# KogarashiNetwork/dusk-plonk

Measured on AMD Instinct MI355X. Metric: PLONK prover constraints/sec (BLS12-381) at n=2^16 and 2^20, 1/2/4/8 GPUs, higher is better.
Workload: dtype u32-limb Montgomery Fr/Fp (integer)

## Files before the change

### dusk-plonk_amd/csrc/debug.hip

```cpp
#include <hip/hip_runtime.h>

#include <algorithm>
#include <vector>

#include "g1r.hpp"
#include "internal.hpp"
#include "prover.hpp"

namespace plk {
namespace {

template <class C>
__global__ void k_field_op(int op, const Fe<C>* __restrict__ a, const Fe<C>* __restrict__ b,
                           Fe<C>* __restrict__ out, uint64_t n) {
  const uint64_t i = (uint64_t)blockIdx.x * blockDim.x + threadIdx.x;
  if (i >= n) return;
  const Fe<C> x = a[i], y = b[i];
  Fe<C> r;
  switch (op) {
    case 0: r = fe_mul(x, y); break;
    case 1: r = fe_add(x, y); break;
    case 2: r = fe_sub(x, y); break;
    case 3: r = fe_sqr(x); break;
    default: r = fe_inv(x); break;
// ... 91 lines not shown
  else if constexpr (OP == kOpSmall2) o0 = rx_small_mul_n<C, 2>(x0);
  else if constexpr (OP == kOpSmall3) o0 = rx_small_mul_n<C, 3>(x0);
  else if constexpr (OP == kOpCanon) o0 = rx_canon(x0);
  else if constexpr (OP == kOpIsZero) o0 = rx_flag<C>(rx_is_zero(x0));
  else if constexpr (OP == kOpIsZeroU) o0 = rx_flag<C>(rx_is_zero_u(x0));
  else if constexpr (OP == kOpUnpackPack) {
    Fe<C> w;
#pragma unroll
    for (int k = 0; k < C::N; ++k) w.v[k] = x0.v[k];
    o0 = rx_unpack(w);
    w = rx_pack(o0);
#pragma unroll
    for (int k = 0; k < C::N; ++k) o1.v[k] = w.v[k];
  } else if constexpr (OP >= kOpSubN) o0 = rx_sub_n<C, OP - kOpSubN>(x0, x1);
  else o0 = rx_sub_u<C, OP - kOpSubU>(x0, x1);
  st_row<C>(out, i * NOUT, o0);
  if constexpr (NOUT > 1) st_row<C>(out, i * NOUT + 1, o1);
  if constexpr (NOUT > 2) st_row<C>(out, i * NOUT + 2, o2);
}

using RxKernel = void (*)(const uint32_t*, const uint32_t*, const uint32_t*, const uint32_t*,
                          uint32_t*, uint64_t);
#define PLK_RX_CASE(C, OP) \
  case OP: return k_rx_op<C, OP>;
#define PLK_RX_COMMON(C)                                                                       \
  PLK_RX_CASE(C, kOpMul) PLK_RX_CASE(C, kOpSqr) PLK_RX_CASE(C, kOpMulAdd) PLK_RX_CASE(C, kOpMul2) \
  PLK_RX_CASE(C, kOpMul2Asm) PLK_RX_CASE(C, kOpSqr2) PLK_RX_CASE(C, kOpMulAddMul2)             \
  PLK_RX_CASE(C, kOpMul3) PLK_RX_CASE(C, kOpAdd) PLK_RX_CASE(C, kOpSub) PLK_RX_CASE(C, kOpSubLazy) \
  PLK_RX_CASE(C, kOpSub2N6) PLK_RX_CASE(C, kOpSmall2) PLK_RX_CASE(C, kOpSmall3)                \
  PLK_RX_CASE(C, kOpCanon) PLK_RX_CASE(C, kOpIsZero) PLK_RX_CASE(C, kOpIsZeroU)                \
  PLK_RX_CASE(C, kOpUnpackPack) PLK_RX_CASE(C, kOpSubU + 3) PLK_RX_CASE(C, kOpSubU + 5)        \
  PLK_RX_CASE(C, kOpSubU + 6) PLK_RX_CASE(C, kOpSubN + 3) PLK_RX_CASE(C, kOpSubN + 5)          \
  PLK_RX_CASE(C, kOpSubN + 6)
RxKernel rx_kernel(int field, int op) {
  if (field == 0) {
    switch (op) {
      PLK_RX_COMMON(FrCfg)
      default: return nullptr;
    }
  }
  switch (op) {
    PLK_RX_COMMON(FpCfg)
    PLK_RX_CASE(FpCfg, kOpSqr2Asm) PLK_RX_CASE(FpCfg, kOpMulAddMul2Asm)
    PLK_RX_CASE(FpCfg, kOpSubU + 4) PLK_RX_CASE(FpCfg, kOpSubU + 10)
    PLK_RX_CASE(FpCfg, kOpSubN + 4) PLK_RX_CASE(FpCfg, kOpSubN + 10)
    default: return nullptr;
  }
}
#undef PLK_RX_COMMON
#undef PLK_RX_CASE

enum : int {
  kG1Madd000 = 0, kG1Madd100, kG1Madd110, kG1Madd111, kG1MaddLazy, kG1AddLazy, kG1AddQuad,
  kG1DblLazy, kG1LazyFinish, kG1Add, kG1AddAffine, kG1Dbl, kG1DblAffine, kG1OpCount
};
constexpr int kG1Row = 4 * RxShape<FpCfg>::L;
constexpr bool g1_op_needs_q(int op) {
  return !(op == kG1DblLazy || op == kG1LazyFinish || op == kG1Dbl || op == kG1DblAffine);
}

__device__ __forceinline__ G1R ld_g1row(const uint32_t* __restrict__ p, uint64_t i) {
  G1R r;
  r.X = ld_row<FpCfg>(p, 4 * i);
  r.Y = ld_row<FpCfg>(p, 4 * i + 1);
  r.ZZ = ld_row<FpCfg>(p, 4 * i + 2);
  r.ZZZ = ld_row<FpCfg>(p, 4 * i + 3);
  return r;
}

template <bool GROUPED, bool ASM, bool PAIRS>
__device__ __forceinline__ G1R madd_as_accumulate(const G1R& acc, const G1R& q, bool neg) {
  RFp y = q.Y;
  if (neg) y = rx_neg_lazy(y);
  const bool was_inf = g1r_is_inf(acc);
  G1R r = g1r_madd_lazy_sl<GROUPED, ASM, PAIRS>(acc, q.X, y);
  if (rx_is_zero(r.ZZ)) {
    RFp yr = q.Y;
    if (neg) yr = rx_neg(yr);
    r = g1r_madd_lazy_fix(was_inf, r, q.X, yr);
  }
  return r;
}

template <int OP>
__global__ void __launch_bounds__(256)
    k_g1r_op(const uint32_t* __restrict__ p, const uint32_t* __restrict__ q,
             const uint32_t* __restrict__ flags, uint32_t* __restrict__ out, uint64_t n) {
  const uint64_t t = (uint64_t)blockIdx.x * blockDim.x + threadIdx.x;
  const uint64_t i = OP == kG1AddQuad ? t >> 2 : t;
  if (i >= n) return;
  const G1R a = ld_g1row(p, i);
  G1R b = g1_op_needs_q(OP) ? ld_g1row(q, i) : a;
  const bool neg = g1_op_needs_q(OP) && flags && (flags[i] & 1u);
  G1R r;
  if constexpr (OP == kG1Madd000) r = madd_as_accumulate<false, false, false>(a, b, neg);
  else if constexpr (OP == kG1Madd100) r = madd_as_accumulate<true, false, false>(a, b, neg);
  else if constexpr (OP == kG1Madd110) r = madd_as_accumulate<true, true, false>(a, b, neg);
  else if constexpr (OP == kG1Madd111) r = madd_as_accumulate<true, true, true>(a, b, neg);
  else if constexpr (OP == kG1MaddLazy) r = g1r_madd_lazy(a, b.X, neg ? rx_neg_lazy(b.Y) : b.Y);
  else if constexpr (OP == kG1AddLazy || OP == kG1AddQuad) {
    if (neg) b.Y = rx_neg_lazy(b.Y);
    if constexpr (OP == kG1AddLazy) r = g1r_add_lazy(a, b);
    else r = g1r_add_quad(a, b, threadIdx.x & 3u);
  } else if constexpr (OP == kG1DblLazy) r = g1r_dbl_lazy(a);
  else if constexpr (OP == kG1LazyFinish) r = g1r_lazy_finish(a);
  else if constexpr (OP == kG1Add) r = g1r_add(a, neg ? g1r_neg(b) : b);
  else if constexpr (OP == kG1AddAffine) r = g1r_add_affine(a, b.X, neg ? rx_neg(b.Y) : b.Y);
  else if constexpr (OP == kG1Dbl) r = g1r_dbl(a);
  else r = g1r_dbl_affine(a.X, a.Y);
  st_row<FpCfg>(out, 4 * t, r.X);
  st_row<FpCfg>(out, 4 * t + 1, r.Y);
  st_row<FpCfg>(out, 4 * t + 2, r.ZZ);
  st_row<FpCfg>(out, 4 * t + 3, r.ZZZ);
}

using G1Kernel = void (*)(const uint32_t*, const uint32_t*, const uint32_t*, uint32_t*, uint64_t);
G1Kernel g1r_kernel(int op) {
  switch (op) {
#define PLK_G1_CASE(OP) \
  case OP: return k_g1r_op<OP>;
    PLK_G1_CASE(kG1Madd000) PLK_G1_CASE(kG1Madd100) PLK_G1_CASE(kG1Madd110)
    PLK_G1_CASE(kG1Madd111) PLK_G1_CASE(kG1MaddLazy) PLK_G1_CASE(kG1AddLazy)
    PLK_G1_CASE(kG1AddQuad) PLK_G1_CASE(kG1DblLazy) PLK_G1_CASE(kG1LazyFinish)
    PLK_G1_CASE(kG1Add) PLK_G1_CASE(kG1AddAffine) PLK_G1_CASE(kG1Dbl) PLK_G1_CASE(kG1DblAffine)
#undef PLK_G1_CASE
    default: return nullptr;
  }
}

struct RowArg {
  const uint32_t* host;
  size_t bytes;
};
template <class K, size_t NA>
int run_rows(plk_ctx* ctx, K kern, const RowArg (&in)[NA], uint32_t* out, size_t out_bytes,
             uint64_t threads, uint64_t n) {
  DevBuf din[NA], dout;
  int st;
  hipStream_t s = ctx->stream;
  for (size_t k = 0; k < NA; ++k) {
    if (!in[k].host) continue;
    if ((st = din[k].alloc(in[k].bytes))) return st;
    PLK_HIP_TRY(hipMemcpyAsync(din[k].ptr, in[k].host, in[k].bytes, hipMemcpyHostToDevice, s));
  }
  if ((st = dout.alloc(out_bytes))) return st;
  const dim3 grid((unsigned)((threads + 255) / 256)), block(256);
  const uint32_t* dp[NA];
  for (size_t k = 0; k < NA; ++k) dp[k] = static_cast<const uint32_t*>(din[k].ptr);
  uint32_t* const dres = static_cast<uint32_t*>(dout.ptr);
  if constexpr (NA == 4)
    hipLaunchKernelGGL(kern, grid, block, 0, s, dp[0], dp[1], dp[2], dp[3], dres, n);
  else
    hipLaunchKernelGGL(kern, grid, block, 0, s, dp[0], dp[1], dp[2], dres, n);
  PLK_HIP_TRY(hipGetLastError());
  PLK_HIP_TRY(hipMemcpyAsync(out, dout.ptr, out_bytes, hipMemcpyDeviceToHost, s));
  PLK_HIP_TRY(stream_wait(s));
  return PLK_OK;
}


enum : int {
  kStPermNumDen = 0, kStScan, kStQuotient, kStPiSparse, kStPiCoef, kStCosetCombine, kStEval,
  kStLinComb, kStScalePowers, kStRuffini, kStCount
};

struct StageCall {
  int stage;
  const uint64_t* const* in;
  const size_t* len;
  size_t n_in;
  const plk_fr* sc;
  size_t n_sc;
  const uint64_t* par;
  size_t n_par;
  uint64_t* out;
  size_t out_cap;
};
// ... 296 lines not shown
```

### dusk-plonk_amd/csrc/ffr.hpp

```cpp
#pragma once
#include <type_traits>
#include <utility>

#include "ff.hpp"

namespace plk {

template <class C>
struct RxShape;
template <>
struct RxShape<FpCfg> {
  static constexpr int L = 13, B = 30;
  static constexpr uint32_t ONE[12] = {0x00d1ff2eu, 0x46760000u, 0x9b4800acu, 0x84b80337u,
                                       0xe882431cu, 0x0dd9a7e0u, 0xb683dcf8u, 0xc26c26d0u,
                                       0x63c4a5eeu, 0x29f14576u, 0x7f3e804bu, 0x015de996u};
};
template <>
struct RxShape<FrCfg> {
  static constexpr int L = 9, B = 29;
  static constexpr uint32_t ONE[8] = {0xffffffbau, 0x00000045u, 0x0072d846u, 0x1a25272eu,
                                      0x5dbeee8bu, 0xfe2eedcdu, 0x9eefbe41u, 0x4d043f42u};
};

template <class C>
// ... 55 lines not shown
  static constexpr int TOP_BITS = 26;
  bool split[2 * L - 1];
  constexpr RxPlan() : split{} {
    constexpr RxConst<C> K = RxK<C>::k;
    long double carry = 0;
    for (int k = 0; k < 2 * L - 1; ++k) {
      long double sum = carry;
      for (int i = 0; i < L; ++i) {
        const int j = k - i;
        if (j < 0 || j >= L) continue;
        const long double ai = (long double)(1ull << (i == L - 1 ? TOP_BITS : B));
        const long double bj = (long double)(1ull << (j == L - 1 ? TOP_BITS : B));
        sum += NPROD * ai * bj + (long double)(1ull << B) * (long double)(K.p[j] + 1);
      }
      split[k] = sum >= 18446744073709551616.0L;
      carry = sum / (long double)(1ull << B) + 4;
    }
  }
};
template <class C, int NPROD>
struct RxPlanK {
  static constexpr RxPlan<C, NPROD> k{};
};
template <class C>
struct RxMultiple {
  uint32_t v[RxShape<C>::L];
};

template <class C>
constexpr RxMultiple<C> rx_multiple(uint32_t c, bool borrow_free) {
  constexpr int L = RxShape<C>::L, B = RxShape<C>::B, N = C::N;
  uint32_t w[N + 1] = {};
  uint64_t carry = 0;
  for (int i = 0; i < N; ++i) {
    const uint64_t t = (uint64_t)C::P[i] * c + carry;
    w[i] = (uint32_t)t;
    carry = t >> 32;
  }
  w[N] = (uint32_t)carry;
  RxMultiple<C> m{};
  for (int i = 0; i < L; ++i) m.v[i] = rx_limb_of(w, N + 1, i, B, L);
  if (borrow_free) {
    m.v[0] += 1u << B;
    for (int i = 1; i < L - 1; ++i) m.v[i] += (1u << B) - 1;
    m.v[L - 1] -= 1;
  }
  return m;
}

template <class C, uint32_t CP, bool BF>
struct RxMultipleK {
  static constexpr RxMultiple<C> k = rx_multiple<C>(CP, BF);
};
static_assert(RxMultiple<FpCfg>{rx_multiple<FpCfg>(12, false)}.v[RxShape<FpCfg>::L - 1] <
                  (1u << RxPlan<FpCfg, 1>::TOP_BITS),
              "12p exceeds the split plan's operand bound");

#define PLK_RX __device__ __forceinline__

PLK_RX void rx_madd(uint64_t& acc, uint32_t x, uint32_t y) { acc += (uint64_t)x * y; }

template <class C>
PLK_RX void rx_column_close(bool split, int k, uint64_t& acc, uint64_t s2, uint64_t s3,
                            uint32_t* m, Rx<C>& r) {
  constexpr int L = RxShape<C>::L, B = RxShape<C>::B;
  constexpr uint32_t MASK = (1u << B) - 1;
  constexpr RxConst<C> K = RxK<C>::k;
  if (!split) {
    if (k < L) {
      m[k] = ((uint32_t)acc * K.inv) & MASK;
      rx_madd(acc, m[k], K.p[0]);
    } else {
      r.v[k - L] = (uint32_t)acc & MASK;
    }
    acc >>= B;
    return;
  }
  const uint32_t lo32 = ((uint32_t)acc & MASK) + ((uint32_t)s2 & MASK) + ((uint32_t)s3 & MASK);
  const uint64_t hi = (acc >> B) + (s2 >> B) + (s3 >> B);
  uint64_t lo = lo32;
  if (k < L) {
    m[k] = (lo32 * K.inv) & MASK;
    lo += (uint64_t)m[k] * K.p[0];
  } else {
    r.v[k - L] = lo32 & MASK;
  }
  acc = hi + (lo >> B);
}

template <class C>
PLK_RX Rx<C> rx_zero() {
  Rx<C> r;
#pragma unroll
  for (int i = 0; i < RxShape<C>::L; ++i) r.v[i] = 0;
  return r;
}

template <class C>
PLK_RX Rx<C> rx_one() {
  constexpr RxConst<C> K = RxK<C>::k;
  Rx<C> r;
#pragma unroll
  for (int i = 0; i < RxShape<C>::L; ++i) r.v[i] = K.one[i];
  return r;
}

template <class C>
// ... 737 lines not shown
```

### dusk-plonk_amd/csrc/g1r.hpp

```cpp
#pragma once
#include "ffr.hpp"
#include "g1.hpp"

namespace plk {

using RFp = Rx<FpCfg>;

struct G1R {
  RFp X, Y, ZZ, ZZZ;
};

__device__ __forceinline__ G1R g1r_infinity() {
  G1R r;
  r.X = rx_one<FpCfg>();
  r.Y = rx_one<FpCfg>();
  r.ZZ = rx_zero<FpCfg>();
  r.ZZZ = rx_zero<FpCfg>();
  return r;
}

__device__ __forceinline__ bool g1r_is_inf(const G1R& p) { return rx_is_zero(p.ZZ); }

__device__ __forceinline__ G1R g1r_neg(const G1R& p) {
  G1R r = p;
// ... 91 lines not shown
    rx_mul2<FpCfg, ASM>(x2, p.ZZ, y2, p.ZZZ, U2, S2);
    const RFp P = rx_sub_u<FpCfg, 10>(U2, p.X);
    const RFp R = rx_sub_u<FpCfg, 6>(S2, p.Y);
    rx_sqr2<FpCfg, ASM>(P, R, PP, RR);
    G1R r;
    rx_mul2<FpCfg, ASM>(P, PP, p.X, PP, PPP, Q);
    r.X = rx_sub2_n<FpCfg, 6>(RR, PPP, Q);
    r.Y = rx_mul_add(R, rx_sub_u<FpCfg, 10>(Q, r.X), rx_sub_u<FpCfg, 5>(rx_zero<FpCfg>(), p.Y), PPP);
    rx_mul2<FpCfg, ASM>(p.ZZ, PP, p.ZZZ, PPP, r.ZZ, r.ZZZ);
    return r;
  } else if constexpr (GROUPED) {
    RFp U2, S2, PP, RR, PPP, Q;
    rx_mul2<FpCfg, ASM>(x2, p.ZZ, y2, p.ZZZ, U2, S2);
    const RFp P = rx_sub_u<FpCfg, 10>(U2, p.X);
    const RFp R = rx_sub_u<FpCfg, 6>(S2, p.Y);
    rx_sqr2<FpCfg, ASM>(P, R, PP, RR);
    G1R r;
    rx_mul2<FpCfg, ASM>(P, PP, p.X, PP, PPP, Q);
    r.X = rx_sub2_n<FpCfg, 6>(RR, PPP, Q);
    rx_mul_add_mul2<FpCfg, ASM>(R, rx_sub_u<FpCfg, 10>(Q, r.X), rx_sub_u<FpCfg, 5>(rx_zero<FpCfg>(), p.Y), PPP,
                    p.ZZ, PP, p.ZZZ, PPP, r.Y, r.ZZ, r.ZZZ);
    return r;
  } else {
    const RFp U2 = rx_mul(x2, p.ZZ);
    const RFp S2 = rx_mul(y2, p.ZZZ);
    const RFp P = rx_sub_u<FpCfg, 10>(U2, p.X);
    const RFp R = rx_sub_u<FpCfg, 6>(S2, p.Y);
    const RFp PP = rx_sqr(P);
    const RFp PPP = rx_mul(P, PP);
    const RFp Q = rx_mul(p.X, PP);
    G1R r;
    r.X = rx_sub2_n<FpCfg, 6>(rx_sqr(R), PPP, Q);
    r.Y = rx_mul_add(R, rx_sub_u<FpCfg, 10>(Q, r.X), rx_sub_u<FpCfg, 5>(rx_zero<FpCfg>(), p.Y), PPP);
    r.ZZ = rx_mul(p.ZZ, PP);
    r.ZZZ = rx_mul(p.ZZZ, PPP);
    return r;
  }
}

__device__ __forceinline__ G1R g1r_madd_lazy_fix(bool was_inf, const G1R& r, const RFp& x2,
                                                 const RFp& y2) {
  if (was_inf) {
    G1R q;
    q.X = x2;
    q.Y = y2;
    q.ZZ = rx_one<FpCfg>();
    q.ZZZ = rx_one<FpCfg>();
    return q;
  }
  if (rx_is_zero_u(r.X)) return g1r_dbl_affine(x2, y2);
  return g1r_infinity();
}

__device__ __forceinline__ G1R g1r_madd_lazy(const G1R& p, const RFp& x2, const RFp& y2) {
  const bool was_inf = g1r_is_inf(p);
  G1R r = g1r_madd_lazy_sl<true>(p, x2, y2);
  if (rx_is_zero(r.ZZ)) r = g1r_madd_lazy_fix(was_inf, r, x2, rx_canon(y2));
  return r;
}

__device__ __forceinline__ RFp rx_neg_lazy(const RFp& y) { return rx_sub_u<FpCfg, 4>(rx_zero<FpCfg>(), y); }

__device__ __forceinline__ G1R g1r_lazy_finish(const G1R& p) {
  G1R r = p;
  r.X = rx_canon(p.X);
  r.Y = rx_canon(p.Y);
  return r;
}

__device__ __forceinline__ G1R g1r_add_lazy_sl(const G1R& p, const G1R& q) {
  RFp U1, U2, ZZ12, S1, S2, ZZZ12, PP, RR, PPP, Q;
  rx_mul3(p.X, q.ZZ, q.X, p.ZZ, p.ZZ, q.ZZ, U1, U2, ZZ12);
  const RFp P = rx_sub_u<FpCfg, 3>(U2, U1);
  rx_mul3(p.Y, q.ZZZ, q.Y, p.ZZZ, p.ZZZ, q.ZZZ, S1, S2, ZZZ12);
  const RFp R = rx_sub_u<FpCfg, 3>(S2, S1);
  rx_sqr2(P, R, PP, RR);
  rx_mul2(P, PP, U1, PP, PPP, Q);
  G1R r;
  r.X = rx_sub2_n<FpCfg, 6>(RR, PPP, Q);
  rx_mul_add_mul2(R, rx_sub_u<FpCfg, 10>(Q, r.X), rx_sub_u<FpCfg, 5>(rx_zero<FpCfg>(), S1), PPP,
                  ZZ12, PP, ZZZ12, PPP, r.Y, r.ZZ, r.ZZZ);
  return r;
}

__device__ __forceinline__ G1R g1r_dbl_lazy(const G1R& p) {
  const RFp U = rx_small_mul_n<FpCfg, 2>(p.Y);
  const RFp V = rx_sqr(U);
  const RFp W = rx_mul(U, V);
  const RFp S = rx_mul(p.X, V);
  const RFp X2 = rx_sqr(p.X);
  const RFp M = rx_small_mul_n<FpCfg, 3>(X2);
  G1R r;
  r.X = rx_sub2_n<FpCfg, 6>(rx_sqr(M), rx_zero<FpCfg>(), S);
  r.Y = rx_mul_add(M, rx_sub_u<FpCfg, 10>(S, r.X), rx_sub_u<FpCfg, 5>(rx_zero<FpCfg>(), p.Y), W);
  r.ZZ = rx_mul(V, p.ZZ);
  r.ZZZ = rx_mul(W, p.ZZZ);
  return r;
}

__device__ __forceinline__ G1R g1r_add_lazy_fix(const G1R& p, const G1R& q, const RFp& x3) {
  if (g1r_is_inf(p)) return q;
  if (g1r_is_inf(q)) return p;
  uint32_t z = 0;
  __asm__ volatile(";; plk rare path" : "+v"(z));
  RFp x = x3;
  x.v[0] += z;
// ... 118 lines not shown
```

### dusk-plonk_amd/csrc/msm.hip

```cpp
#include <hip/hip_ext.h>
#include <hip/hip_runtime.h>

#include <algorithm>
#include <cstdlib>
#include <cstring>
#include <vector>

#include "internal.hpp"
#include "msm_common.hpp"
#include "g1r.hpp"

namespace plk {

namespace {

#ifndef PLK_LANE_PARTIALS
#define PLK_LANE_PARTIALS 4
#endif
#ifndef PLK_CHUNK_TARGET
#define PLK_CHUNK_TARGET 262144
#endif
constexpr uint32_t kHistThreads = 1024;
constexpr uint32_t kHistBlocksMax = 256;

// ... 463 lines not shown
      run += s_len[l];
    }
    if (blockIdx.x == 0) {
      offsets[B] = s_c[nt - 1];
      task_off[B] = s_t[nt - 1];
    }
  }
  __syncthreads();
  uint32_t c_run = s_c[tid] - c_sum, t_run = s_t[tid] - t_sum, f_run = s_f[tid] - f_sum;
  for (uint32_t b = b0; b < b1; ++b) {
    const uint32_t cnt = s_count[b];
    if (b >= bl && b < bh) {
      s_count[b] = c_run;
      offsets[b] = c_run;
      task_off[b] = t_run;
      const uint32_t nfull = cnt / chunk, tail = cnt - nfull * chunk;
      for (uint32_t t = 0; t < nfull; ++t)
        tasks[f_run + t] = make_uint2(c_run + t * chunk, (t_run + t) | ((chunk - 1) << kTaskShift));
      if (tail)
        tasks[atomicAdd(&s_cur[tail], 1u)] =
            make_uint2(c_run + nfull * chunk, (t_run + nfull) | ((tail - 1) << kTaskShift));
    }
    c_run += cnt;
    t_run += (cnt + chunk - 1) / chunk;
    f_run += cnt / chunk;
  }
  __syncthreads();
  auto scatter_digits = [&](const Fr& x, bool neg, uint32_t i) {
    each_digit<C>(x, cfg, [&](uint32_t w, int d) {
      const uint32_t b = (uint32_t)(d < 0 ? -d : d) - 1u;
      if (b - bl < bpart) {
        const uint32_t pos = atomicAdd(&s_count[b], 1u);
        out[pos] = (uint32_t)(w * n_srs + i) | (((d < 0) != neg) ? 0x80000000u : 0u);
      }
    });
  };
  if constexpr (HOLD) {
#pragma unroll
    for (uint32_t k = 0; k < kPer; ++k) {
      const uint32_t i = tid + k * nt;
      if (i >= len) break;
      scatter_digits(sv[k], sneg[k], i);
    }
  } else {
    for_scalars(sc, 0, len, tid, nt,
                [&](uint32_t i, const Fr& x, bool neg) { scatter_digits(x, neg, i); });
  }
}

constexpr uint32_t kFineBits = 10;
constexpr uint32_t kFineBitsMin = 8;
constexpr uint32_t kCoarseMax = 4096;
constexpr uint32_t kRunBits = 4, kRunBitsMin = 1;
constexpr size_t kRunLanes = 65536;
inline size_t run_lanes() {
  static const size_t v = [] {
    const char* e = getenv("PLK_RUN_LANES");
    const long long x = e ? atoll(e) : 0;
    return x > 0 ? (size_t)x : kRunLanes;
  }();
  return v;
}
inline uint32_t batch_run_bits() {
  static const uint32_t v = [] {
    const char* e = getenv("PLK_RUN_BITS_BATCH");
    const int x = e ? atoi(e) : 0;
    return x >= 1 && x <= 8 ? (uint32_t)x : kRunBits;
  }();
  return v;
}
inline uint32_t run_bits(uint32_t B, uint32_t slots) {
  if (slots > 1) return std::min<uint32_t>(batch_run_bits(), 31 - __builtin_clz(B));
  uint32_t rb = kRunBits;
  while (rb > kRunBitsMin && (size_t)(B >> rb) < run_lanes()) --rb;
  return rb;
}

template <int K>
__device__ __forceinline__ void block_scan_excl(uint32_t (&v)[K], uint32_t (&tot)[K], uint32_t* sh) {
  const uint32_t lane = threadIdx.x & 63, wid = threadIdx.x >> 6, nw = blockDim.x >> 6;
  uint32_t inc[K];
#pragma unroll
  for (int k = 0; k < K; ++k) inc[k] = v[k];
#pragma unroll
  for (uint32_t o = 1; o < 64; o <<= 1) {
#pragma unroll
    for (int k = 0; k < K; ++k) {
      const uint32_t t = __shfl_up(inc[k], o, 64);
      if (lane >= o) inc[k] += t;
    }
  }
  if (lane == 63) {
#pragma unroll
    for (int k = 0; k < K; ++k) sh[k * 32 + wid] = inc[k];
  }
  __syncthreads();
#pragma unroll
  for (int k = 0; k < K; ++k) {
    uint32_t base = 0, total = 0;
    for (uint32_t w = 0; w < nw; ++w) {
      const uint32_t s = sh[k * 32 + w];
      base += w < wid ? s : 0u;
      total += s;
    }
    v[k] = base + inc[k] - v[k];
    tot[k] = total;
// ... 232 lines not shown
    else return g1r_add_t<LAZY>(a, b);
  }
  __device__ __forceinline__ G1R down(const G1R& v, uint32_t h) const { return shfl_down_g1r(v, h * S); }
  template <bool LAZY>
  __device__ __forceinline__ G1R tree(G1R acc, uint32_t e, uint32_t w) const {
    for (uint32_t h = w >> 1; h >= 1; h >>= 1) {
      const G1R o = down(acc, h);
      if (e < h) acc = add<LAZY>(acc, o);
    }
    return acc;
  }
};

#ifndef PLK_BITSUM_WAVES
#define PLK_BITSUM_WAVES 2
#endif

template <bool QUAD>
__global__ void __launch_bounds__(256) k_bucket_sum(const uint32_t* __restrict__ task_off,
                                                    uint32_t B, uint32_t lp, uint64_t task_stride,
                                                    const G1xyzz* __restrict__ partials,
                                                    G1xyzz* __restrict__ bsum) {
  const uint32_t slot = blockIdx.y;
  const TailUnit<QUAD> T(blockIdx.x * 256 + threadIdx.x);
  const uint32_t P = 1u << lp, s = T.u & (P - 1);
  const uint32_t b = T.u >> lp;
  task_off += (size_t)slot * (B + 1);
  partials += (size_t)slot * task_stride;
  G1R acc = g1r_infinity();
  if (b < B)
    for (uint32_t t = task_off[b] + s; t < task_off[b + 1]; t += P) acc = T.template add<false>(acc, ld_g1r(&partials[t]));
  acc = T.template tree<false>(acc, s, P);
  if (s == 0 && T.l == 0 && b < B) st_g1r(&bsum[(size_t)slot * B + b], QUAD ? g1r_lazy_finish(acc) : acc);
}

#ifndef PLK_RUNSUM_WAVES
#define PLK_RUNSUM_WAVES 1
#endif
__global__ void __launch_bounds__(256, PLK_RUNSUM_WAVES) k_runsum1(const uint32_t* __restrict__ task_off, uint32_t B, uint32_t rb,
                                                 uint64_t task_stride,
                                                 const G1xyzz* __restrict__ partials,
                                                 G1xyzz* __restrict__ rsum) {
  const uint32_t K = 1u << rb;
  const uint32_t slot = blockIdx.y, NR = B >> rb;
  const uint32_t r = blockIdx.x * blockDim.x + threadIdx.x;
  if (r >= NR) return;
  task_off += (size_t)slot * (B + 1);
  partials += (size_t)slot * task_stride;
  rsum += (size_t)slot * B;
  __shared__ G1xyzz s_prev[256];
  G1xyzz* prev = &s_prev[threadIdx.x];
  G1R R = g1r_infinity();
  uint32_t pe = task_off[r * K + K];
  for (uint32_t t = K; t-- > 0;) {
    const uint32_t b = r * K + t;
    const uint32_t p0 = task_off[b];
    for (uint32_t p = p0; p < pe; ++p) {
      st_g1r(prev, R);
      G1R c = g1r_add_lazy_sl(R, ld_g1r(&partials[p]));
      if (rx_is_zero(c.ZZ)) c = g1r_add_lazy_fix(ld_g1r(prev), ld_g1r(&partials[p]), c.X);
      R = c;
    }
    pe = p0;
    st_g1r(&rsum[b], R);
  }
}

__global__ void __launch_bounds__(256, PLK_RUNSUM_WAVES) k_runsum2(uint32_t B, uint32_t rb, const G1xyzz* __restrict__ rsum,
                                                 G1xyzz* __restrict__ ys, G1xyzz* __restrict__ ts) {
  const uint32_t K = 1u << rb;
  const uint32_t slot = blockIdx.y, NR = B >> rb;
  const uint32_t r = blockIdx.x * blockDim.x + threadIdx.x;
  if (r >= NR) return;
  rsum += (size_t)slot * B + (size_t)r * K;
  __shared__ G1xyzz s_prev[256];
  G1xyzz* prev = &s_prev[threadIdx.x];
  G1R T = ld_g1r(&rsum[0]);
  for (uint32_t t = 1; t < K; ++t) {
    const G1R v = ld_g1r(&rsum[t]);
    if (g1r_is_inf(v)) continue;
    st_g1r(prev, T);
    G1R c = g1r_add_lazy_sl(T, v);
    if (rx_is_zero(c.ZZ)) c = g1r_add_lazy_fix(ld_g1r(prev), ld_g1r(&rsum[t]), c.X);
    T = c;
  }
  st_g1r(&ys[(size_t)slot * NR + r], g1r_lazy_finish(ld_g1r(&rsum[0])));
  st_g1r(&ts[(size_t)slot * NR + r], g1r_lazy_finish(T));
}

constexpr uint32_t kBitsumOut = 10;

struct BitsumFold {
  uint32_t* done;
  G1xyzz* out2;
  const uint32_t* offsets;
  uint32_t* entries;
  uint32_t B, nbits, nout;
};
constexpr uint32_t kFoldMaxGroups = 16;

__device__ __forceinline__ uint32_t with_bit(uint32_t k, uint32_t j) {
  return ((k >> j) << (j + 1)) | (1u << j) | (k & ((1u << j) - 1u));
}

constexpr uint32_t bitsum1_threads(bool z, bool quad) {
  return quad ? 512 : (z ? 192 : 128);
}
template <bool Z, bool QUAD>
__global__ void __launch_bounds__(bitsum1_threads(Z, QUAD), PLK_BITSUM_WAVES) k_bitsum1(uint32_t B, const G1xyzz* __restrict__ bsum,
                                                                           const G1xyzz* __restrict__ zin,
                                                                           G1xyzz* __restrict__ out,
                                                                           BitsumFold fold) {
  constexpr uint32_t NS = Z ? 48 : 32;
  constexpr bool SPLIT = Z && QUAD;
  constexpr uint32_t NSU = 4, MEM = 16 / NSU;
  constexpr uint32_t NU = bitsum1_threads(Z, QUAD) / TailUnit<QUAD>::S;
  constexpr bool LZ = false;
  __shared__ G1xyzz sh[NS];
  const uint32_t slot = blockIdx.y, g = blockIdx.x, tid = threadIdx.x;
  const uint32_t role = SPLIT ? blockIdx.z : 0;
  const TailUnit<QUAD> T(tid);
  out += ((size_t)slot * gridDim.x + g) * kBitsumOut;
  auto value = [&](uint32_t x) -> G1R {
    const uint32_t b = g * 256 + (x & 255);
    const G1xyzz* src = x < 256 ? bsum : zin;
    return b < B ? ld_g1r(&src[(size_t)slot * B + b]) : g1r_infinity();
// ... 397 lines not shown
      PLK_SORT_ONE_LAUNCH(false);
    }
#undef PLK_SORT_ONE_LAUNCH
  } else {
    const size_t lds = (size_t)std::min<uint32_t>(B, kLdsBuckets) * 4;
    if (max_len) {
      PLK_BY_C(s->c, hipLaunchKernelGGL(k_hist<CC>, dim3(hist_blocks, slots), dim3(kHistThreads), lds,
                                        stream, batch, cfg, w.blockhist.as<uint32_t>()))
    } else {
      PLK_HIP_TRY(hipMemsetAsync(w.blockhist.ptr, 0, (size_t)slots * hist_blocks * B * 4, stream));
    }
    const bool small_sort = B <= kSortSmallMax;
    if (small_sort) {
      hipLaunchKernelGGL(k_sort_small, dim3(1, slots), dim3(1024), 0, stream,
                         w.blockhist.as<uint32_t>(), hist_blocks, B, chunk, w.offsets.as<uint32_t>(),
                         w.task_off.as<uint32_t>(), w.tasks.as<uint2>(), (uint64_t)w.task_stride);
    } else {
      hipLaunchKernelGGL(k_block_scan, dim3(cdiv(B, 256), slots), dim3(256), 0, stream,
                         w.blockhist.as<uint32_t>(), hist_blocks, B, w.counts.as<uint32_t>(),
                         (uint32_t*)nullptr, (uint32_t*)nullptr);
      hipLaunchKernelGGL(k_scan_buckets, dim3(1, slots), dim3(1024), (size_t)B * 4, stream,
                         w.counts.as<uint32_t>(), B, chunk, w.offsets.as<uint32_t>(),
                         w.task_off.as<uint32_t>(), w.full_off.as<uint32_t>(),
                         w.len_cur.as<uint32_t>());
    }
    if (max_len) {
      PLK_BY_C(s->c, hipLaunchKernelGGL(k_scatter<CC>, dim3(hist_blocks, slots), dim3(kHistThreads),
                                        lds, stream, batch, cfg, (uint64_t)s->n,
                                        w.offsets.as<uint32_t>(), w.blockhist.as<uint32_t>(),
                                        w.sorted.as<uint32_t>(), (uint64_t)w.sorted_stride))
    }
    if (!small_sort) {
      hipLaunchKernelGGL(k_make_tasks, dim3(cdiv(B, 256), slots), dim3(256), 0, stream,
                         w.offsets.as<uint32_t>(), w.task_off.as<uint32_t>(),
                         w.full_off.as<uint32_t>(), w.len_cur.as<uint32_t>(), B, chunk,
                         w.tasks.as<uint2>(), (uint64_t)w.task_stride);
    }
  }
  if (guard_limit) {
    hipLaunchKernelGGL(k_guard, dim3(std::min<uint32_t>(64, cdiv(B, 1024)), slots), dim3(256), 0, stream,
                       (const uint32_t*)w.offsets.as<uint32_t>(), w.task_off.as<uint32_t>(), B,
                       guard_limit, w.guard.as<uint32_t>(), hdr_dev->max_count);
  }
  const int tail = w.tail_quad;
  const bool quad = tail == 1;
  launch_accumulate(s->has_inf, !w.shared_chip, dim3(cdiv(max_tasks_used, 256), slots), stream, w.ev0, w.ev1,
                    w.tasks.as<uint2>(), w.task_off.as<uint32_t>(), B, (uint64_t)w.task_stride,
                    w.sorted.as<uint32_t>(), (uint64_t)w.sorted_stride, s->table.as<G1Affine>(),
                    s->table_inf.as<uint8_t>(), w.partials.as<G1xyzz>());
  if (wide) {
    hipLaunchKernelGGL(k_runsum1, dim3(cdiv(NR, 256), slots), dim3(256), 0, stream,
                       (const uint32_t*)w.task_off.as<uint32_t>(), B, rb, (uint64_t)w.task_stride,
                       (const G1xyzz*)w.partials.as<G1xyzz>(), w.rsum.as<G1xyzz>());
    hipLaunchKernelGGL(k_runsum2, dim3(cdiv(NR, 256), slots), dim3(256), 0, stream, B, rb,
                       (const G1xyzz*)w.rsum.as<G1xyzz>(), w.ys.as<G1xyzz>(), w.zs.as<G1xyzz>());
  } else {
    const size_t per_bucket = cdiv(total_entries, (size_t)chunk * B * slots) + 1;
    uint32_t lp = 0;
    while (lp < 4 && ((size_t)PLK_LANE_PARTIALS << lp) < per_bucket && (((size_t)B * slots) << lp) < 131072) ++lp;
    if (quad) {
      hipLaunchKernelGGL(k_bucket_sum<true>, dim3(cdiv(((size_t)B << lp) * 4, 256), slots), dim3(256), 0, stream,
                         w.task_off.as<uint32_t>(), B, lp, (uint64_t)w.task_stride,
                         w.partials.as<G1xyzz>(), w.bsum.as<G1xyzz>());
    } else {
      hipLaunchKernelGGL(k_bucket_sum<false>, dim3(cdiv((size_t)B << lp, 256), slots), dim3(256), 0, stream,
                         w.task_off.as<uint32_t>(), B, lp, (uint64_t)w.task_stride,
                         w.partials.as<G1xyzz>(), w.bsum.as<G1xyzz>());
    }
  }
  BitsumFold fold{};
  if (G <= kFoldMaxGroups) {
    fold.done = w.done.as<uint32_t>();
    fold.out2 = bits_dev;
    fold.offsets = w.offsets.as<uint32_t>();
    fold.entries = hdr_dev->entries;
    fold.B = B;
    fold.nbits = nbits;
    fold.nout = nout;
  }
  if (quad) bitsum_launch<true, true>(wide, G, slots, NR, B, w, fold, nbits, nout, bits_dev, hdr_dev, stream);
  else if (tail == 2) bitsum_launch<false, true>(wide, G, slots, NR, B, w, fold, nbits, nout, bits_dev, hdr_dev, stream);
  else bitsum_launch<false, false>(wide, G, slots, NR, B, w, fold, nbits, nout, bits_dev, hdr_dev, stream);
  PLK_HIP_TRY(hipGetLastError());

  const ReadbackHeader* hdr = w.host_out.as<ReadbackHeader>();
  const G1xyzz* T = reinterpret_cast<const G1xyzz*>(hdr + 1);
  PLK_HIP_TRY(stream_wait(stream));
  const uint32_t* ent = hdr->entries;
  uint32_t flag[kMaxSlots];
  for (uint32_t k = 0; k < slots; ++k) flag[k] = hdr->flag[k] == gen ? 1u : 0u;
  MsmStats& stt = w.stats;
  float ms = 0.f;
  if (hipEventElapsedTime(&ms, w.ev0, w.ev1) == hipSuccess) stt.last_accumulate_ms = ms;
  bool hot[kMaxSlots] = {};
  for (uint32_t k = 0; k < slots; ++k) {
    hot[k] = guard_limit && hdr->max_count[k] > guard_limit;
    if (info) info[k] = MsmSlotInfo{ent[k], guard_limit ? hdr->max_count[k] : 0u, hot[k]};
  }
  stt.last_point_adds = 0;
  for (uint32_t k = 0; k < slots; ++k) stt.last_point_adds += hot[k] ? 0u : ent[k];
  stt.last_slots = slots;
  stt.cum_accumulate_ms += stt.last_accumulate_ms;
  stt.cum_launches += 1;
  stt.cum_point_adds += stt.last_point_adds;
  for (uint32_t k = 0; k < slots; ++k) stt.cum_points += batch.len[k];

  int overall = PLK_OK;
// ... 55 lines not shown
```

### dusk-plonk_amd/csrc/msm_acc.hip

```cpp
#include <hip/hip_ext.h>
#include <hip/hip_runtime.h>

#include "internal.hpp"
#include "msm_common.hpp"
#include "g1r.hpp"


namespace plk {

namespace {

constexpr uint32_t kAccThreads = 256;

typedef __attribute__((address_space(3))) void lds_void;

__device__ __forceinline__ void stage_point(const G1Affine* p, uint4 (*stage)[64]) {
  const uint4* q = reinterpret_cast<const uint4*>(p);
#pragma unroll
  for (int i = 0; i < 6; ++i)
    __builtin_amdgcn_global_load_lds((const void*)(q + i), (lds_void*)&stage[i][0], 16, 0, 0);
}

__device__ __forceinline__ void unstage_point(const uint4 (*stage)[64], uint32_t lane, RFp& x,
                                              RFp& y) {
  Fp px, py;
#pragma unroll
  for (int i = 0; i < 3; ++i) {
    const uint4 a = stage[i][lane], b = stage[i + 3][lane];
    px.v[4 * i] = a.x; px.v[4 * i + 1] = a.y; px.v[4 * i + 2] = a.z; px.v[4 * i + 3] = a.w;
    py.v[4 * i] = b.x; py.v[4 * i + 1] = b.y; py.v[4 * i + 2] = b.z; py.v[4 * i + 3] = b.w;
  }
  x = rx_unpack(px);
  y = rx_unpack(py);
}

template <bool HAS_INF, bool LONE>
__global__ void __launch_bounds__(kAccThreads)
    __attribute__((amdgpu_waves_per_eu(LONE ? 3 : 2, LONE ? 3 : 2)))
    k_accumulate(const uint2* __restrict__ tasks, const uint32_t* __restrict__ task_off, uint32_t B,
                 uint64_t task_stride, const uint32_t* __restrict__ sorted, uint64_t sorted_stride,
                 const G1Affine* __restrict__ table, const uint8_t* __restrict__ table_inf,
                 G1xyzz* __restrict__ partials) {
  const uint32_t slot = blockIdx.y;
  const uint32_t t = blockIdx.x * blockDim.x + threadIdx.x;
  __shared__ uint4 s_stage[kAccThreads / 64][6][64];
  uint4 (*stage)[64] = s_stage[threadIdx.x >> 6];
  const uint32_t lane = threadIdx.x & 63;
  if (t >= task_off[(size_t)slot * (B + 1) + B]) return;
  const uint2 tk = tasks[(size_t)slot * task_stride + t];
  const uint2 task = make_uint2(tk.x, (tk.y >> kTaskShift) + 1);
  const uint32_t pidx = tk.y & ((1u << kTaskShift) - 1);
  sorted += (size_t)slot * sorted_stride;
  const uint32_t end = task.x + task.y;
  G1R acc = g1r_infinity();
  {
    const uint32_t c0 = sorted[task.x];
    if (!HAS_INF || !table_inf[c0 & 0x7fffffffu]) {
      ld_g1r_aff(&table[c0 & 0x7fffffffu], acc.X, acc.Y);
      if (c0 & 0x80000000u) acc.Y = rx_neg(acc.Y);
      acc.ZZ = rx_one<FpCfg>();
      acc.ZZZ = rx_one<FpCfg>();
    }
  }
  uint32_t code = task.x + 1 < end ? sorted[task.x + 1] : 0u;
  bool inf = HAS_INF && task.x + 1 < end && table_inf[code & 0x7fffffffu];
  if (task.x + 1 < end) stage_point(&table[code & 0x7fffffffu], stage);
  uint32_t next = task.x + 2 < end ? sorted[task.x + 2] : 0u;
  for (uint32_t e = task.x + 1; e < end; ++e) {
    const uint32_t cur = code;
    const bool cur_inf = inf;
    RFp x, y;
    unstage_point(stage, lane, x, y);
    __asm__ volatile("s_waitcnt lgkmcnt(0)" ::: "memory");
    if (e + 1 < end) {
      code = next;
      if (HAS_INF) inf = table_inf[code & 0x7fffffffu];
      stage_point(&table[code & 0x7fffffffu], stage);
      if (e + 2 < end) next = sorted[e + 2];
    }
    if (HAS_INF && cur_inf) continue;
    if (cur & 0x80000000u) y = rx_neg_lazy(y);
    const bool was_inf = g1r_is_inf(acc);
    G1R r = g1r_madd_lazy_sl<true, true, LONE>(acc, x, y);
    if (rx_is_zero(r.ZZ)) {
      RFp xr, yr;
      ld_g1r_aff(&table[cur & 0x7fffffffu], xr, yr);
      if (cur & 0x80000000u) yr = rx_neg(yr);
      r = g1r_madd_lazy_fix(was_inf, r, xr, yr);
    }
    acc = r;
  }
  st_g1r(&partials[(size_t)slot * task_stride + pidx], g1r_lazy_finish(acc));
}

}

void launch_accumulate(bool has_inf, bool lone, dim3 grid, hipStream_t stream, hipEvent_t ev0,
                       hipEvent_t ev1, const uint2* tasks, const uint32_t* task_off, uint32_t B,
                       uint64_t task_stride, const uint32_t* sorted, uint64_t sorted_stride,
                       const G1Affine* table, const uint8_t* table_inf, G1xyzz* partials) {
  const dim3 block(kAccThreads);
#define PLK_ACC_LAUNCH(I, L)                                                                   \
  hipExtLaunchKernelGGL((k_accumulate<I, L>), grid, block, 0, stream, ev0, ev1, 0, tasks, task_off, \
                        B, task_stride, sorted, sorted_stride, table, table_inf, partials)
  if (has_inf) {
    if (lone) PLK_ACC_LAUNCH(true, true);
    else PLK_ACC_LAUNCH(true, false);
  } else {
    if (lone) PLK_ACC_LAUNCH(false, true);
    else PLK_ACC_LAUNCH(false, false);
  }
#undef PLK_ACC_LAUNCH
}

}
```

### dusk-plonk_amd/plonk.py

```python
from __future__ import annotations

import ctypes as C
import os
from pathlib import Path

import numpy as np

_PKG = Path(__file__).resolve().parent
_LIB_PATH = Path(os.environ["PLK_LIB"]) if os.environ.get("PLK_LIB") else _PKG / "libplk.so"

PLK_OK, PLK_E_DEGREE, PLK_E_ARG, PLK_E_DEVICE, PLK_E_OOM, PLK_E_NODEV = range(6)

_SRS_IO_SYMBOLS = (
    "plk_srs_load_bytes", "plk_srs_export_bytes", "plk_srs_last_load_ms", "plk_srs_fold",
    "plk_srs_verify", "plk_srs_last_verify_ms", "plk_opening_key_load_bytes",
    "plk_opening_key_to_bytes", "plk_debug_srs_weights", "plk_debug_f2_sqrt",
)

_SRS_UPDATE_SYMBOLS = (
    "plk_g1_mul_batch", "plk_g1_mul_last_ms", "plk_opening_key_update", "plk_srs_update",
    "plk_srs_verify_update", "plk_g2_to_bytes", "plk_g2_from_bytes", "plk_debug_glv_split",
)

_CHECK_SYMBOLS = ("plk_composer_check", "plk_prover_diagnose", "plk_key_diagnose", "plk_check_last_ms")
# ... 219 lines not shown
class Context:

    _default: dict[int, "Context"] = {}

    def __init__(self, device: int = 0):
        h = C.c_void_p()
        _check(_lib().plk_ctx_create(device, C.byref(h)), "plk_ctx_create")
        self.handle = h
        self.device = device
        self._domains: dict[int, C.c_void_p] = {}

    @classmethod
    def default(cls, device: int | None = None) -> "Context":
        if device is None:
            device = int(os.environ.get("LOCAL_RANK", "0")) if "LOCAL_RANK" in os.environ else 0
            try:
                import torch
                if torch.cuda.is_available():
                    device = torch.cuda.current_device()
            except Exception:
                pass
        if device not in cls._default:
            cls._default[device] = Context(device)
        return cls._default[device]

    def stream(self) -> int:
        s = C.c_void_p()
        _check(_lib().plk_ctx_stream(self.handle, C.byref(s)), "plk_ctx_stream")
        return s.value or 0

    def synchronize(self):
        _check(_lib().plk_ctx_synchronize(self.handle), "plk_ctx_synchronize")

    def field_op(self, field: str, op: str, a: np.ndarray, b: np.ndarray | None = None):
        w = 4 if field == "fr" else 6
        a = np.ascontiguousarray(np.asarray(a, dtype=np.uint64).reshape(-1, w))
        bb = None if b is None else np.ascontiguousarray(np.asarray(b, dtype=np.uint64).reshape(-1, w))
        out = np.zeros_like(a)
        code = {"mul": 0, "add": 1, "sub": 2, "sqr": 3, "inv": 4}[op]
        _check(_lib().plk_debug_field_op(self.handle, 0 if field == "fr" else 1, code, _ptr(a),
                                         None if bb is None else _ptr(bb), _ptr(out), a.shape[0]),
               "plk_debug_field_op")
        return out

    RX_OPS = {"mul": (0, 2, 1), "sqr": (1, 1, 1), "mul_add": (2, 4, 1), "mul2": (3, 4, 2),
              "mul2_asm": (4, 4, 2), "sqr2": (5, 2, 2), "sqr2_asm": (6, 2, 2),
              "mul_add_mul2": (7, 4, 3), "mul_add_mul2_asm": (8, 4, 3), "mul3": (9, 4, 3),
              "add": (10, 2, 1), "sub": (11, 2, 1), "sub_lazy": (12, 2, 1), "sub2_n6": (13, 3, 1),
              "small_mul2": (14, 1, 1), "small_mul3": (15, 1, 1), "canon": (16, 1, 1),
              "is_zero": (17, 1, 1), "is_zero_u": (18, 1, 1), "unpack_pack": (19, 1, 2),
              "sub_u": (100, 2, 1), "sub_n": (200, 2, 1)}
    G1R_OPS = {"madd_000": 0, "madd_100": 1, "madd_110": 2, "madd_111": 3, "madd_lazy": 4,
               "add_lazy": 5, "add_quad": 6, "dbl_lazy": 7, "lazy_finish": 8, "add": 9,
               "add_affine": 10, "dbl": 11, "dbl_affine": 12}

    def rx_op(self, field: str, op: str, *rows, cp: int = 0) -> np.ndarray:
        L = 9 if field == "fr" else 13
        code, nin, nout = self.RX_OPS[op]
        if len(rows) != nin:
            raise ValueError(f"rx_op {op} takes {nin} operand arrays")
        ops = [np.ascontiguousarray(np.asarray(r, dtype=np.uint32).reshape(-1, L)) for r in rows]
        n = ops[0].shape[0]
        if any(o.shape[0] != n for o in ops):
            raise ValueError("rx_op operands differ in length")
        out = np.zeros((n, nout, L), dtype=np.uint32)
        ptrs = [_ptr(o) for o in ops] + [None] * (4 - nin)
        _check(_lib().plk_debug_rx_op(self.handle, 0 if field == "fr" else 1, code + cp, *ptrs,
                                      _ptr(out), n), "plk_debug_rx_op")
        return out

    NTT_LAZY_OPS = {"reduce_q": (0, 1, 1), "add_u": (1, 2, 1), "sub_u": (2, 2, 1),
                    "sub_u2_11": (3, 2, 1), "r4": (4, 7, 4), "r4_h1": (5, 5, 4),
                    "r2first": (6, 3, 2), "odd_last": (7, 2, 2), "store0": (8, 1, 1),
                    "store1": (9, 2, 1), "store2": (10, 2, 1)}

    def ntt_lazy_op(self, op: str, *rows) -> np.ndarray:
        code, nin, nout = self.NTT_LAZY_OPS[op]
        if len(rows) != nin:
            raise ValueError(f"ntt_lazy_op {op} takes {nin} operand arrays")
        ops = [np.asarray(r, dtype=np.uint32).reshape(-1, 9) for r in rows]
        n = ops[0].shape[0]
        if any(o.shape[0] != n for o in ops):
            raise ValueError("ntt_lazy_op operands differ in length")
        cases = np.ascontiguousarray(np.stack(ops, axis=1))
        out = np.zeros((n, nout, 9), dtype=np.uint32)
        _check(_lib().plk_debug_ntt_lazy_op(self.handle, code, _ptr(cases), _ptr(out), n),
               "plk_debug_ntt_lazy_op")
        return out

    def g1r_op(self, op: str, p, q=None, flags=None) -> np.ndarray:
        p = np.ascontiguousarray(np.asarray(p, dtype=np.uint32).reshape(-1, 4, 13))
        n = p.shape[0]
        if q is not None:
            q = np.ascontiguousarray(np.asarray(q, dtype=np.uint32).reshape(-1, 4, 13))
        if flags is not None:
            flags = np.ascontiguousarray(np.asarray(flags, dtype=np.uint32).reshape(-1))
        if any(x is not None and x.shape[0] != n for x in (q, flags)):
            raise ValueError("g1r_op operands differ in length")
        out = np.zeros((n, 4, 4, 13) if op == "add_quad" else (n, 4, 13), dtype=np.uint32)
        _check(_lib().plk_debug_g1r_op(self.handle, self.G1R_OPS[op], _ptr(p),
                                       None if q is None else _ptr(q),
                                       None if flags is None else _ptr(flags), _ptr(out), n),
               "plk_debug_g1r_op")
        return out

    PROVER_STAGES = {"perm_numden": 0, "scan": 1, "quotient": 2, "pi_sparse": 3, "pi_coef": 4,
                     "coset_combine": 5, "eval": 6, "lincomb": 7, "scale_powers": 8, "ruffini": 9}
# ... 819 lines not shown
```

Before: 35.56 million.

## Add affine+affine first-step bucket add and skip empty running-sum slots

Adds a specialised affine+affine lazy point addition and uses it for the first accumulation step in the MSM bucket accumulator, where the accumulator is still affine (ZZ=ZZZ=1), avoiding the general mixed-add multiplications. Running-sum kernels now start from the first partial rather than adding to infinity, and for sparse slots they early-exit or write infinity when a run has no tasks. Debug ops and Python bindings are added for testing the new formula. Risks include correctness edge cases (doubling or infinity in the first step) and extra branches and task_off reads in the runsum kernels.

```diff
diff --git a/dusk-plonk_amd/csrc/debug.hip b/dusk-plonk_amd/csrc/debug.hip
--- a/dusk-plonk_amd/csrc/debug.hip
+++ b/dusk-plonk_amd/csrc/debug.hip
@@ -167,7 +167,8 @@
 
 enum : int {
   kG1Madd000 = 0, kG1Madd100, kG1Madd110, kG1Madd111, kG1MaddLazy, kG1AddLazy, kG1AddQuad,
-  kG1DblLazy, kG1LazyFinish, kG1Add, kG1AddAffine, kG1Dbl, kG1DblAffine, kG1OpCount
+  kG1DblLazy, kG1LazyFinish, kG1Add, kG1AddAffine, kG1Dbl, kG1DblAffine, kG1AddAffAff,
+  kG1AddAffAffAsm, kG1OpCount
 };
 constexpr int kG1Row = 4 * RxShape<FpCfg>::L;
 constexpr bool g1_op_needs_q(int op) {
@@ -194,6 +195,13 @@
     if (neg) yr = rx_neg(yr);
     r = g1r_madd_lazy_fix(was_inf, r, q.X, yr);
   }
+  return r;
+}
+
+template <bool ASM>
+__device__ __forceinline__ G1R aff_aff_as_accumulate(const G1R& a, const G1R& q, bool neg) {
+  G1R r = g1r_add_aff_aff_lazy_sl<ASM>(a.X, a.Y, q.X, neg ? rx_neg_lazy(q.Y) : q.Y);
+  if (rx_is_zero(r.ZZ)) r = g1r_madd_lazy_fix(false, r, q.X, neg ? rx_neg(q.Y) : q.Y);
   return r;
 }
 
@@ -222,6 +230,8 @@
   else if constexpr (OP == kG1Add) r = g1r_add(a, neg ? g1r_neg(b) : b);
   else if constexpr (OP == kG1AddAffine) r = g1r_add_affine(a, b.X, neg ? rx_neg(b.Y) : b.Y);
   else if constexpr (OP == kG1Dbl) r = g1r_dbl(a);
+  else if constexpr (OP == kG1AddAffAff) r = aff_aff_as_accumulate<false>(a, b, neg);
+  else if constexpr (OP == kG1AddAffAffAsm) r = aff_aff_as_accumulate<true>(a, b, neg);
   else r = g1r_dbl_affine(a.X, a.Y);
   st_row<FpCfg>(out, 4 * t, r.X);
   st_row<FpCfg>(out, 4 * t + 1, r.Y);
@@ -238,6 +248,7 @@
     PLK_G1_CASE(kG1Madd111) PLK_G1_CASE(kG1MaddLazy) PLK_G1_CASE(kG1AddLazy)
     PLK_G1_CASE(kG1AddQuad) PLK_G1_CASE(kG1DblLazy) PLK_G1_CASE(kG1LazyFinish)
     PLK_G1_CASE(kG1Add) PLK_G1_CASE(kG1AddAffine) PLK_G1_CASE(kG1Dbl) PLK_G1_CASE(kG1DblAffine)
+    PLK_G1_CASE(kG1AddAffAff) PLK_G1_CASE(kG1AddAffAffAsm)
 #undef PLK_G1_CASE
     default: return nullptr;
   }
diff --git a/dusk-plonk_amd/csrc/ffr.hpp b/dusk-plonk_amd/csrc/ffr.hpp
--- a/dusk-plonk_amd/csrc/ffr.hpp
+++ b/dusk-plonk_amd/csrc/ffr.hpp
@@ -131,7 +131,8 @@
 struct RxMultipleK {
   static constexpr RxMultiple<C> k = rx_multiple<C>(CP, BF);
 };
-static_assert(RxMultiple<FpCfg>{rx_multiple<FpCfg>(12, false)}.v[RxShape<FpCfg>::L - 1] <
+constexpr uint32_t kRxOperandBoundP = 12;
+static_assert(RxMultiple<FpCfg>{rx_multiple<FpCfg>(kRxOperandBoundP, false)}.v[RxShape<FpCfg>::L - 1] <
                   (1u << RxPlan<FpCfg, 1>::TOP_BITS),
               "12p exceeds the split plan's operand bound");
 
diff --git a/dusk-plonk_amd/csrc/g1r.hpp b/dusk-plonk_amd/csrc/g1r.hpp
--- a/dusk-plonk_amd/csrc/g1r.hpp
+++ b/dusk-plonk_amd/csrc/g1r.hpp
@@ -167,6 +167,22 @@
   return g1r_infinity();
 }
 
+static_assert(3 + 4 <= kRxOperandBoundP && 10 + 2 <= kRxOperandBoundP,
+              "g1r_add_aff_aff_lazy_sl's multiplicands exceed the split plan's operand bound");
+template <bool ASM = false>
+__device__ __forceinline__ G1R g1r_add_aff_aff_lazy_sl(const RFp& x1, const RFp& y1, const RFp& x2,
+                                                       const RFp& y2) {
+  const RFp P = rx_sub_u<FpCfg, 3>(x2, x1);
+  const RFp R = rx_sub_u<FpCfg, 3>(y2, y1);
+  RFp RR, Q;
+  G1R r;
+  rx_sqr2<FpCfg, ASM>(P, R, r.ZZ, RR);
+  rx_mul2<FpCfg, ASM>(P, r.ZZ, x1, r.ZZ, r.ZZZ, Q);
+  r.X = rx_sub2_n<FpCfg, 6>(RR, r.ZZZ, Q);
+  r.Y = rx_mul_add(R, rx_sub_u<FpCfg, 10>(Q, r.X), rx_sub_u<FpCfg, 5>(rx_zero<FpCfg>(), y1), r.ZZZ);
+  return r;
+}
+
 __device__ __forceinline__ G1R g1r_madd_lazy(const G1R& p, const RFp& x2, const RFp& y2) {
   const bool was_inf = g1r_is_inf(p);
   G1R r = g1r_madd_lazy_sl<true>(p, x2, y2);
diff --git a/dusk-plonk_amd/csrc/msm.hip b/dusk-plonk_amd/csrc/msm.hip
--- a/dusk-plonk_amd/csrc/msm.hip
+++ b/dusk-plonk_amd/csrc/msm.hip
@@ -539,6 +539,7 @@
 constexpr uint32_t kFineBitsMin = 8;
 constexpr uint32_t kCoarseMax = 4096;
 constexpr uint32_t kRunBits = 4, kRunBitsMin = 1;
+constexpr uint32_t kSparseSlotTasks = 1u << 12;
 constexpr size_t kRunLanes = 65536;
 inline size_t run_lanes() {
   static const size_t v = [] {
@@ -877,10 +878,17 @@
   G1xyzz* prev = &s_prev[threadIdx.x];
   G1R R = g1r_infinity();
   uint32_t pe = task_off[r * K + K];
+  if (task_off[B] < kSparseSlotTasks && task_off[r * K] == pe) return;
+  bool started = false;
   for (uint32_t t = K; t-- > 0;) {
     const uint32_t b = r * K + t;
     const uint32_t p0 = task_off[b];
-    for (uint32_t p = p0; p < pe; ++p) {
+    uint32_t p = p0;
+    if (!started && p < pe) {
+      R = ld_g1r(&partials[p++]);
+      started = true;
+    }
+    for (; p < pe; ++p) {
       st_g1r(prev, R);
       G1R c = g1r_add_lazy_sl(R, ld_g1r(&partials[p]));
       if (rx_is_zero(c.ZZ)) c = g1r_add_lazy_fix(ld_g1r(prev), ld_g1r(&partials[p]), c.X);
@@ -891,12 +899,20 @@
   }
 }
 
-__global__ void __launch_bounds__(256, PLK_RUNSUM_WAVES) k_runsum2(uint32_t B, uint32_t rb, const G1xyzz* __restrict__ rsum,
+__global__ void __launch_bounds__(256, PLK_RUNSUM_WAVES) k_runsum2(const uint32_t* __restrict__ task_off, uint32_t B, uint32_t rb,
+                                                 const G1xyzz* __restrict__ rsum,
                                                  G1xyzz* __restrict__ ys, G1xyzz* __restrict__ ts) {
   const uint32_t K = 1u << rb;
   const uint32_t slot = blockIdx.y, NR = B >> rb;
   const uint32_t r = blockIdx.x * blockDim.x + threadIdx.x;
   if (r >= NR) return;
+  task_off += (size_t)slot * (B + 1);
+  if (task_off[B] < kSparseSlotTasks && task_off[r * K] == task_off[r * K + K]) {
+    const G1R inf = g1r_lazy_finish(g1r_infinity());
+    st_g1r(&ys[(size_t)slot * NR + r], inf);
+    st_g1r(&ts[(size_t)slot * NR + r], inf);
+    return;
+  }
   rsum += (size_t)slot * B + (size_t)r * K;
   __shared__ G1xyzz s_prev[256];
   G1xyzz* prev = &s_prev[threadIdx.x];
@@ -1400,7 +1416,8 @@
     hipLaunchKernelGGL(k_runsum1, dim3(cdiv(NR, 256), slots), dim3(256), 0, stream,
                        (const uint32_t*)w.task_off.as<uint32_t>(), B, rb, (uint64_t)w.task_stride,
                        (const G1xyzz*)w.partials.as<G1xyzz>(), w.rsum.as<G1xyzz>());
-    hipLaunchKernelGGL(k_runsum2, dim3(cdiv(NR, 256), slots), dim3(256), 0, stream, B, rb,
+    hipLaunchKernelGGL(k_runsum2, dim3(cdiv(NR, 256), slots), dim3(256), 0, stream,
+                       (const uint32_t*)w.task_off.as<uint32_t>(), B, rb,
                        (const G1xyzz*)w.rsum.as<G1xyzz>(), w.ys.as<G1xyzz>(), w.zs.as<G1xyzz>());
   } else {
     const size_t per_bucket = cdiv(total_entries, (size_t)chunk * B * slots) + 1;
diff --git a/dusk-plonk_amd/csrc/msm_acc.hip b/dusk-plonk_amd/csrc/msm_acc.hip
--- a/dusk-plonk_amd/csrc/msm_acc.hip
+++ b/dusk-plonk_amd/csrc/msm_acc.hip
@@ -66,10 +66,9 @@
   bool inf = HAS_INF && task.x + 1 < end && table_inf[code & 0x7fffffffu];
   if (task.x + 1 < end) stage_point(&table[code & 0x7fffffffu], stage);
   uint32_t next = task.x + 2 < end ? sorted[task.x + 2] : 0u;
-  for (uint32_t e = task.x + 1; e < end; ++e) {
-    const uint32_t cur = code;
-    const bool cur_inf = inf;
-    RFp x, y;
+  auto take_entry = [&](uint32_t e, uint32_t& cur, bool& cur_inf, RFp& x, RFp& y) {
+    cur = code;
+    cur_inf = inf;
     unstage_point(stage, lane, x, y);
     __asm__ volatile("s_waitcnt lgkmcnt(0)" ::: "memory");
     if (e + 1 < end) {
@@ -78,6 +77,37 @@
       stage_point(&table[code & 0x7fffffffu], stage);
       if (e + 2 < end) next = sorted[e + 2];
     }
+  };
+  uint32_t e = task.x + 1;
+  if (e < end) {
+    uint32_t cur;
+    bool cur_inf;
+    RFp x, y;
+    take_entry(e, cur, cur_inf, x, y);
+    ++e;
+    if (HAS_INF && cur_inf) {
+    } else if (HAS_INF && g1r_is_inf(acc)) {
+      acc.X = x;
+      acc.Y = (cur & 0x80000000u) ? rx_neg(y) : y;
+      acc.ZZ = rx_one<FpCfg>();
+      acc.ZZZ = rx_one<FpCfg>();
+    } else {
+      if (cur & 0x80000000u) y = rx_neg_lazy(y);
+      G1R r = g1r_add_aff_aff_lazy_sl<true>(acc.X, acc.Y, x, y);
+      if (rx_is_zero(r.ZZ)) {
+        RFp xr, yr;
+        ld_g1r_aff(&table[cur & 0x7fffffffu], xr, yr);
+        if (cur & 0x80000000u) yr = rx_neg(yr);
+        r = g1r_madd_lazy_fix(false, r, xr, yr);
+      }
+      acc = r;
+    }
+  }
+  for (; e < end; ++e) {
+    uint32_t cur;
+    bool cur_inf;
+    RFp x, y;
+    take_entry(e, cur, cur_inf, x, y);
     if (HAS_INF && cur_inf) continue;
     if (cur & 0x80000000u) y = rx_neg_lazy(y);
     const bool was_inf = g1r_is_inf(acc);
diff --git a/dusk-plonk_amd/plonk.py b/dusk-plonk_amd/plonk.py
--- a/dusk-plonk_amd/plonk.py
+++ b/dusk-plonk_amd/plonk.py
@@ -295,7 +295,8 @@
               "sub_u": (100, 2, 1), "sub_n": (200, 2, 1)}
     G1R_OPS = {"madd_000": 0, "madd_100": 1, "madd_110": 2, "madd_111": 3, "madd_lazy": 4,
                "add_lazy": 5, "add_quad": 6, "dbl_lazy": 7, "lazy_finish": 8, "add": 9,
-               "add_affine": 10, "dbl": 11, "dbl_affine": 12}
+               "add_affine": 10, "dbl": 11, "dbl_affine": 12, "add_aff_aff": 13,
+               "add_aff_aff_asm": 14}
 
     def rx_op(self, field: str, op: str, *rows, cp: int = 0) -> np.ndarray:
         L = 9 if field == "fr" else 13
```

New measurement: 35.95 million, median of 2. Within noise of the previous version (+1.1%).
